# shao-lab/MotifScan

Hardware: AMD Instinct MI355X
Metric: scanned bp*motifs per second (region_bp x n_motifs), both strands, p=1e-4 cutoffs (higher is better)
Workload: dtype f64 (every hit decision and score, as in the reference) behind an fp6 x fp4 one-hot matrix-core pre-filter (exact f32 accumulate)

## Files before the change

include/motifscan_amd.h:

```cpp
#ifndef MOTIFSCAN_AMD_H
#define MOTIFSCAN_AMD_H

#include <stdint.h>

#ifdef __cplusplus
extern "C" {
#endif

#define MS_OK            0
#define MS_ERR_INVALID   1
#define MS_ERR_NOMEM     2
#define MS_ERR_RUNTIME   3

#define MS_STRAND_FWD    1
#define MS_STRAND_REV    2
#define MS_STRAND_BOTH   3

#define MS_SCAN_DEFAULT      0u
#define MS_SCAN_EXACT_ONLY   1u
#define MS_SCAN_COUNTS_ONLY  2u

typedef struct ms_pwmset ms_pwmset;
typedef struct ms_seqset ms_seqset;
typedef struct ms_result ms_result;
// ... 9 lines not shown
    int32_t n_tiles;
    int32_t n_passes;
    double  ms_prefilter;
    double  ms_exact;
    double  ms_sort;
    double  ms_finalize;
    double  ms_total;
    int64_t lds_bytes_read;
    int64_t hbm_bytes_algorithmic;
    double  pf_clock_mhz;
    int64_t mfma_ops;
    int64_t mfma_ops_algorithmic;
    int32_t pf_engine;
    int32_t order_overflow_runs;
    int32_t order_bucketed;
    int32_t reserved0;
} ms_scan_stats;

const char *ms_last_error(void);
int ms_version(void);

int ms_device_count(int *count);
int ms_set_device(int device);
int ms_device_name(char *buf, int buflen);
int ms_numa_bind_thread(int force, int *node);
int ms_device_pool_stats(uint64_t out[6]);

int ms_pwmset_create(const double *values, const int32_t *widths, const double *cutoffs,
                     int32_t n_pwms, ms_pwmset **out);
int ms_pwmset_set_cutoffs(ms_pwmset *pwms, const double *cutoffs);
int ms_pwmset_size(const ms_pwmset *pwms, int32_t *n_pwms);
// ... 161 lines not shown
```

include/motifscan_amd_debug.h:

```cpp
#ifndef MOTIFSCAN_AMD_DEBUG_H
#define MOTIFSCAN_AMD_DEBUG_H

#include "motifscan_amd.h"

#ifdef __cplusplus
extern "C" {
#endif

int ms_debug_plan_dims(const ms_pwmset *pwms, int strand_mask, int64_t lds_budget, int32_t *n_fast,
                       int32_t *n_exact, int32_t *n_groups, int32_t *n_tiles);

int ms_debug_plan_rows(const ms_pwmset *pwms, int32_t *group_fields, int16_t *rows, int32_t *bias, int32_t *group_kb,
                       int32_t *exact_motifs, int32_t *tile_first_group);

int ms_debug_host_pack(const char *bases, const int64_t *offsets, int64_t n_seqs, uint32_t *codes, uint32_t *nmask, int32_t *blk2reg, int32_t *blkinfo);

int ms_debug_numa_probe(const char *root, const char *bdf, int32_t *node, int32_t *n_cpus, int32_t *n_nodes);

int ms_debug_bucket_plan(const int64_t *offsets, int64_t n_seqs, const int32_t *widths, int32_t n_pwms, int32_t gbits, int32_t pbits, int32_t end_bit,
                         int32_t low_bits, int64_t n_regions, uint64_t *weights, double mu, uint64_t n_pred, uint64_t cap_max, uint32_t form, int32_t force,
                         uint64_t *need, int32_t *gate, uint64_t *base, uint64_t *cap);

int ms_debug_key_layout(int64_t n_bases, int64_t n_seqs, int64_t max_len, int32_t n_pwms, int32_t coord_global, int32_t *gbits, int32_t *pbits);

int ms_debug_release_scratch(void);

int ms_debug_varscan_chunk(int64_t n_variants, int64_t *previous);

int ms_debug_best_segment_windows(void);

int ms_debug_pair_lds_bins(void);
int ms_debug_cooc_chunk_regions(void);
int ms_debug_pair_lds_pair_limit(int64_t limit, int64_t *previous);

int ms_debug_plot_dims(int32_t out[6]);

// ... 11 lines not shown
```

motifscan_amd/_lib.py:

```python
import ctypes
import importlib.util
import os
import subprocess

import numpy as np

_HERE = os.path.dirname(os.path.abspath(__file__))
LIB_PATH = os.path.join(_HERE, "libmotifscan_amd.so")

MS_OK, MS_ERR_INVALID, MS_ERR_NOMEM, MS_ERR_RUNTIME = 0, 1, 2, 3
MS_SCAN_DEFAULT, MS_SCAN_EXACT_ONLY, MS_SCAN_COUNTS_ONLY = 0, 1, 2
MS_STREAM_DEDUP, MS_STREAM_NO_HITS, MS_STREAM_EXACT_ONLY, MS_STREAM_PACKED, MS_STREAM_HOST_PACK, MS_STREAM_PACKED12 = 1, 2, 4, 8, 16, 32
MS_PROFILE_UNSMOOTHED = 1
MS_REPLAY_DONE, MS_REPLAY_WORDS, MS_REPLAY_ATTEMPTS, MS_REPLAY_NO_SIZE, MS_REPLAY_EMPTY_RANGE, MS_REPLAY_WIDE = 0, 1, 2, 3, 4, 5
MS_REPLAY_SIZE_MISSING = -(1 << 63)


class ScanStats(ctypes.Structure):
    _fields_ = [("n_bases", ctypes.c_int64), ("n_windows", ctypes.c_int64), ("n_candidates", ctypes.c_int64),
                ("n_hits", ctypes.c_int64), ("n_pwms", ctypes.c_int32), ("n_pwms_exact", ctypes.c_int32),
                ("n_tiles", ctypes.c_int32), ("n_passes", ctypes.c_int32), ("ms_prefilter", ctypes.c_double),
                ("ms_exact", ctypes.c_double), ("ms_sort", ctypes.c_double), ("ms_finalize", ctypes.c_double),
                ("ms_total", ctypes.c_double), ("lds_bytes_read", ctypes.c_int64),
                ("hbm_bytes_algorithmic", ctypes.c_int64), ("pf_clock_mhz", ctypes.c_double),
                ("mfma_ops", ctypes.c_int64), ("mfma_ops_algorithmic", ctypes.c_int64), ("pf_engine", ctypes.c_int32),
                ("order_overflow_runs", ctypes.c_int32), ("order_bucketed", ctypes.c_int32), ("reserved0", ctypes.c_int32)]

    def as_dict(self):
        return {k: getattr(self, k) for k, _ in self._fields_}


class Span(ctypes.Structure):
    _fields_ = [("chrom", ctypes.c_int32), ("reserved", ctypes.c_int32), ("begin", ctypes.c_int64), ("end", ctypes.c_int64),
                ("first_window", ctypes.c_int64), ("n_windows", ctypes.c_int64)]


_lib = None


def build(verbose=False):
    cmd = ["make", "-C", os.path.join(_HERE, "csrc"), "-j4"]
# ... 133 lines not shown
        "ms_allelescan_num_sites": (c_int, [vp, pi64]),
        "ms_allelescan_motif_offsets": (c_int, [vp, pi64]),
        "ms_allelescan_sites": (c_int, [vp, pi64, pu8, pi64, pi8, pd]),
        "ms_allelescan_motif_counts": (c_int, [vp, pi64, pi64]),
        "ms_allelescan_ref_mismatch": (c_int, [vp, pu8]),
        "ms_allelescan_device_ms": (c_int, [vp, pd]),
        "ms_allelescan_free": (None, [vp]),
        "ms_scan_best": (c_int, [vp, vp, c_int, c_u32, pvp]),
        "ms_best_shape": (c_int, [vp, pi32, pi64]),
        "ms_best_sites": (c_int, [vp, c_i32, c_i32, pd, pi32, pi8]),
        "ms_best_sites_device": (c_int, [vp, pvp, pvp, pvp]),
        "ms_best_device_ms": (c_int, [vp, pd]),
        "ms_best_free": (None, [vp]),
        "ms_debug_best_segment_windows": (c_int, []),
        "ms_debug_key_layout": (c_int, [c_i64, c_i64, c_i64, c_i32, c_i32, pi32, pi32]),
    }
    for name, (res, args) in sig.items():
        fn = getattr(L, name)
        fn.restype, fn.argtypes = res, args
    _lib = L
    return L


def check(rc):
    if rc == MS_OK:
        return
    msg = lib().ms_last_error().decode("utf-8", "replace")
    if rc == MS_ERR_INVALID:
        raise ValueError(msg)
    if rc == MS_ERR_NOMEM:
# ... 584 lines not shown
    base, cap = np.zeros(256, dtype=np.uint64), np.zeros(256, dtype=np.uint64)
    form = (1 if predicted else 0) | (2 if counts_only else 0) | (4 if carry_only else 0) | (8 if sticky_off else 0)
    check(lib().ms_debug_bucket_plan(po, n_seqs, pw, n_pwms, int(gbits), int(pbits), int(end_bit), int(low_bits), int(n_regions), ptr(w, ctypes.c_uint64), float(mu),
                                     int(n_pred), (1 << 64) - 1 if cap_max is None else int(cap_max), form, int(force), ctypes.byref(need),
                                     ctypes.byref(gate), ptr(base, ctypes.c_uint64), ptr(cap, ctypes.c_uint64)))
    return {"weights": w, "need": need.value, "gate": bool(gate.value), "base": base, "cap": cap}


def key_layout(n_bases, n_seqs, max_len, n_pwms, coord_global=False):
    gbits, pbits = ctypes.c_int32(), ctypes.c_int32()
    check(lib().ms_debug_key_layout(int(n_bases), int(n_seqs), int(max_len), int(n_pwms), 1 if coord_global else 0, ctypes.byref(gbits),
                                    ctypes.byref(pbits)))
    return gbits.value, pbits.value


def host_pack(bases, offsets):
    bases = np.ascontiguousarray(bases, dtype=np.uint8)
    offsets = np.ascontiguousarray(offsets, dtype=np.int64)
    n = int(offsets[-1])
    units, blocks = (n + 31) // 32, (n + 63) // 64 + 1
    codes, nmask = np.zeros(2 * units, dtype=np.uint32), np.zeros(units, dtype=np.uint32)
    blk, info = np.zeros(blocks, dtype=np.int32), np.zeros((blocks, 4), dtype=np.int32)
    check(lib().ms_debug_host_pack(bases.ctypes.data_as(ctypes.c_char_p), ptr(offsets, ctypes.c_int64), offsets.size - 1,
                                   ptr(codes, ctypes.c_uint32), ptr(nmask, ctypes.c_uint32), ptr(blk, ctypes.c_int32), ptr(info, ctypes.c_int32)))
    return codes, nmask, blk, info


def host_pool_stats():
    out = (ctypes.c_uint64 * 4)()
    check(lib().ms_host_pool_stats(out))
# ... 518 lines not shown
```

motifscan_amd/csrc/ms_fp64.hip:

```cpp
#include "ms_device.h"

namespace ms {

__device__ __forceinline__ int64_t hit_coord(const HitOut &H, const DevSeq &S, int64_t r, int64_t g) {
    return H.pbits ? (int64_t) (((uint64_t) r << H.pbits) | (uint64_t) (g - S.offsets[r])) : g;
}

__device__ __forceinline__ void emit_hit(const HitOut &H, uint32_t motif, int64_t g, uint32_t sbit, double score) {
    const unsigned long long i = atomicAdd(H.n_hits, 1ULL);
    if (i < H.cap) {
        H.keys[i] = ((uint64_t) motif << (H.gbits + 1)) | ((uint64_t) g << 1) | sbit;
        H.vals[i] = score;
    }
}

__device__ __forceinline__ void test_and_emit(const HitOut &H, const DevPwm &Pw, uint32_t motif, int64_t g,
                                              double fwd, double rev, int strand_mask) {
    const double floor_ = Pw.raw_floor[motif];
    const bool try_f = (strand_mask & 1) && !(fwd < floor_);
    const bool try_r = (strand_mask & 2) && !(rev < floor_);
    if (!try_f && !try_r) return;
    const double max_raw = Pw.max_raw[motif];
    const double cutoff = Pw.cutoff[motif];
    const double s_f = try_f ? fwd / max_raw : 0.0, s_r = try_r ? rev / max_raw : 0.0;
// ... 35 lines not shown

template <class ST>
__device__ __forceinline__ void stage_flush(ST &st, const HitOut &H) {
    __syncthreads();
    const unsigned int n = st.n < (unsigned int) ST::kCap ? st.n : (unsigned int) ST::kCap;
    if (threadIdx.x == 0 && n > 0) st.base = atomicAdd(H.n_hits, (unsigned long long) n);
    __syncthreads();
    const unsigned long long base = st.base;
    for (unsigned int i = threadIdx.x; i < n; i += blockDim.x)
        if (base + i < H.cap) { H.keys[base + i] = st.keys[i]; H.vals[base + i] = st.vals[i]; }
    __syncthreads();
    if (threadIdx.x == 0) st.n = 0;
    __syncthreads();
}

template <class ST, class HO>
__device__ __forceinline__ void test_and_stage(ST &st, const HO &H, const DevPwm &Pw, uint32_t motif, int64_t g,
                                               double fwd, double rev, int strand_mask, float floor32) {
    const double floor_ = (double) floor32;
    const bool try_f = (strand_mask & 1) && !(fwd < floor_);
    const bool try_r = (strand_mask & 2) && !(rev < floor_);
    if (!try_f && !try_r) return;
    const double2 mc = *reinterpret_cast<const double2 *>(Pw.thresh + 4 * (size_t) motif);
    const double max_raw = mc.x, cutoff = mc.y;
    if (try_f) {
        const double s = fwd / max_raw;
        if (s - cutoff >= -1e-10) stage_hit(st, H, motif, g, 0u, s);
    }
    if (try_r) {
        const double s = rev / max_raw;
        if (s - cutoff >= -1e-10) stage_hit(st, H, motif, g, 1u, s);
    }
}

__global__ void __launch_bounds__(256) exact_all_kernel(const DevSeq S, const DevPwm Pw, const int32_t *__restrict__ motifs,
                                                        int strand_mask, const HitOut H) {
    const int64_t g = (int64_t) blockIdx.x * blockDim.x + threadIdx.x;
    if (g >= S.n_bases) return;
// ... 160 lines not shown
                       field_meta, strand_mask, H);
    MS_HIP(hipGetLastError());
    return MS_OK;
}

constexpr int kRwThreads = 1024;
constexpr int kRwPerThread = 4;
constexpr int kRwChunk = kRwThreads * kRwPerThread;
constexpr int kRwBins = 4096;
typedef HitStageN<2048> RwStage;
struct RwStageBk : RwStage {
    unsigned int cnt[kOrderBuckets], room[kOrderBuckets];
    unsigned long long lo[kOrderBuckets];
};

__device__ __forceinline__ void stage_flush(RwStageBk &st, const BucketHitOut &H) {
    constexpr int kPer = RwStageBk::kCap / kRwThreads;
    static_assert(kPer * kRwThreads == RwStageBk::kCap && kOrderBuckets <= kRwThreads, "stage_flush: one pass of the block over the stage");
    __syncthreads();
    const unsigned int n = st.n < (unsigned int) RwStageBk::kCap ? st.n : (unsigned int) RwStageBk::kCap;
    if (threadIdx.x < (unsigned int) kOrderBuckets) st.cnt[threadIdx.x] = 0;
    __syncthreads();
    uint32_t bk[kPer], rank[kPer];
#pragma unroll
    for (int k = 0; k < kPer; k++) {
        const unsigned int i = threadIdx.x + (unsigned int) (k * kRwThreads);
        bk[k] = i < n ? (uint32_t) (st.keys[i] >> H.B.shift) & 255u : 0u;
        rank[k] = i < n ? atomicAdd(&st.cnt[bk[k]], 1u) : 0u;
    }
    __syncthreads();
// ... 7 lines not shown
    }
    __syncthreads();
#pragma unroll
    for (int k = 0; k < kPer; k++) {
        const unsigned int i = threadIdx.x + (unsigned int) (k * kRwThreads);
        if (i < n && rank[k] < st.room[bk[k]]) {
            const unsigned long long at = st.lo[bk[k]] + rank[k];
            if (at < H.cap) { H.keys[at] = st.keys[i]; H.vals[at] = st.vals[i]; }
        }
    }
    __syncthreads();
    if (threadIdx.x == 0) st.n = 0;
    __syncthreads();
}

template <class HO, class ST>
__global__ void __launch_bounds__(kRwThreads) rescore_carry_kernel(const DevSeq S, const DevPwm Pw, const uint64_t *__restrict__ cand,
                                                                   const unsigned long long *__restrict__ n_cand, uint64_t n_static, uint64_t cand_cap,
                                                                   const FieldMeta *__restrict__ field_meta, int strand_mask, const HO H) {
    extern __shared__ uint4 rw_lds4[];
    uint64_t *s_cw = reinterpret_cast<uint64_t *>(rw_lds4);
    uint64_t *s_gk = s_cw + kRwChunk;
    uint32_t *s_nw = reinterpret_cast<uint32_t *>(s_gk + kRwChunk);
    uint32_t *s_gf = s_nw + kRwChunk;
    uint32_t *bins = s_gf + kRwChunk;
    uint32_t *wave_tot = bins + kRwBins;
    ST &st = *reinterpret_cast<ST *>(wave_tot + 32);
    if (threadIdx.x == 0) st.n = 0;
    unsigned long long n = n_static + *n_cand;
    if (n > cand_cap) n = cand_cap;
    const bool both = strand_mask == 3;
    const int4 *__restrict__ meta4 = reinterpret_cast<const int4 *>(field_meta);
    const uint32_t lane = threadIdx.x & 63u, wave = threadIdx.x >> 6;
    const uint64_t pmask = H.pbits ? ((1ULL << H.pbits) - 1ULL) : 0ULL;
    const unsigned long long n_chunks = (n + kRwChunk - 1) / kRwChunk;
    for (unsigned long long ch = blockIdx.x; ch < n_chunks; ch += gridDim.x) {
        for (uint32_t i = threadIdx.x; i < (uint32_t) kRwBins; i += kRwThreads) bins[i] = 0;
        __syncthreads();
        {
            uint64_t cw[kRwPerThread], gk[kRwPerThread];
            uint32_t nw[kRwPerThread], gf[kRwPerThread], key[kRwPerThread], rank[kRwPerThread];
            int64_t g[kRwPerThread];
            int4 bi[kRwPerThread];
#pragma unroll
            for (int k = 0; k < kRwPerThread; k++) {
                const unsigned long long i = ch * kRwChunk + (unsigned long long) k * kRwThreads + threadIdx.x;
                const uint64_t rec = i < n ? cand[i] : 0ULL;
                g[k] = (int64_t) (rec >> 30);
                gf[k] = (uint32_t) rec & 0x3FFFFFFFu;
                if (!(gf[k] & 0xFFFFu)) { gf[k] = 0; g[k] = 0; }
                bi[k] = S.blkinfo[g[k] >> 6];
                cw[k] = code_window(S.codes, g[k]);
                nw[k] = n_window(S.nmask, g[k]);
            }
#pragma unroll
            for (int k = 0; k < kRwPerThread; k++) {
                const int64_t base = g[k] & ~(int64_t) 63;
                int64_t lo = bi[k].x, o0 = base + bi[k].y, o1 = base + bi[k].z, o2 = base + bi[k].w, r, beg, end;
                if (bi[k].x < 0) {
                    lo = S.blk2reg[g[k] >> 6];
                    o0 = S.offsets[lo]; o1 = S.offsets[lo + 1];
                    o2 = lo + 2 <= S.R ? S.offsets[lo + 2] : o1;
                }
                if (g[k] < o1) { r = lo; beg = o0; end = o1; }
                else if (g[k] < o2) { r = lo + 1; beg = o1; end = o2; }
                else { r = find_region(S, g[k]); beg = S.offsets[r]; end = S.offsets[r + 1]; }
                const uint64_t coord = H.pbits ? (((uint64_t) r << H.pbits) | (uint64_t) (g[k] - beg)) : (uint64_t) g[k];
                const int64_t room = end - g[k];
                gk[k] = (coord << 8) | (uint64_t) (room > 255 ? 255 : (room < 0 ? 0 : room));
                const uint32_t f = gf[k] & 0xFFFFu;
                const uint32_t fl = both ? (f | (f >> 1)) & 0x5555u : f;
                key[k] = fl ? (((gf[k] >> 16) << 4) | (uint32_t) (__ffs((int) fl) - 1)) & (uint32_t) (kRwBins - 1) : (uint32_t) (kRwBins - 1);
            }
#pragma unroll
            for (int k = 0; k < kRwPerThread; k++) rank[k] = atomicAdd(&bins[key[k]], 1u);
            __syncthreads();
            {
                const uint32_t b0 = bins[4 * threadIdx.x], b1 = bins[4 * threadIdx.x + 1], b2 = bins[4 * threadIdx.x + 2], b3 = bins[4 * threadIdx.x + 3];
                const uint32_t tot = b0 + b1 + b2 + b3;
                uint32_t v = tot;
#pragma unroll
                for (int d = 1; d < 64; d <<= 1) {
                    const uint32_t o = __shfl_up(v, d);
                    if ((int) lane >= d) v += o;
                }
                if (lane == 63u) wave_tot[wave] = v;
                __syncthreads();
                uint32_t base = 0;
                for (uint32_t w = 0; w < wave; w++) base += wave_tot[w];
                const uint32_t excl = base + v - tot;
                bins[4 * threadIdx.x] = excl;
                bins[4 * threadIdx.x + 1] = excl + b0;
                bins[4 * threadIdx.x + 2] = excl + b0 + b1;
                bins[4 * threadIdx.x + 3] = excl + b0 + b1 + b2;
            }
            __syncthreads();
#pragma unroll
            for (int k = 0; k < kRwPerThread; k++) {
                const uint32_t at = bins[key[k]] + rank[k];
                s_cw[at] = cw[k]; s_gk[at] = gk[k]; s_nw[at] = nw[k]; s_gf[at] = gf[k];
            }
        }
        __syncthreads();
        for (int round = 0; round < 2; round++) {
#pragma unroll
            for (int u = 0; u < 2; u++) {
                const uint32_t at = (uint32_t) (round * 2 + u) * kRwThreads + threadIdx.x;
                const uint32_t gfu = s_gf[at];
                const uint32_t f = gfu & 0xFFFFu;
                uint32_t flags = both ? (f | (f >> 1)) & 0x5555u : f;
                if (!flags) continue;
                const uint64_t cwu = s_cw[at], gku = s_gk[at];
                const uint32_t nwu = s_nw[at];
                const int32_t group = (int32_t) (gfu >> 16);
                const int room = (int) (gku & 0xFFu);
                const int64_t coord = (int64_t) (gku >> 8);
                while (flags) {
                    const int field = __ffs((int) flags) - 1;
                    flags &= flags - 1u;
                    const int4 f4 = meta4[group * kGroupFields + field];
                    const int32_t m = f4.x;
                    const int w = f4.y;
                    if (m < 0) continue;
                    if (w > room) continue;
                    double fwd, rev;
                    if (w <= 32 && Pw.tab32) score_window32(Pw.tab2, (uint32_t) f4.z, Pw.zero_bytes, w, cwu, nwu, fwd, rev);
                    else {
                        const int64_t gpos = H.pbits ? S.offsets[coord >> H.pbits] + (int64_t) ((uint64_t) coord & pmask) : coord;
                        score_window(S, Pw.tab2 + Pw.tab_off[m], w, gpos, fwd, rev);
                    }
                    test_and_stage(st, H, Pw, (uint32_t) m, coord, fwd, rev, strand_mask, __int_as_float(f4.w));
                }
            }
            stage_flush(st, H);
        }
    }
}

template <class ST>
static size_t rescore_carry_lds_bytes() { return (size_t) kRwChunk * 24 + (size_t) kRwBins * 4 + 32 * 4 + sizeof(ST) + 64; }
int rescore_carry_set_lds() {
    MS_HIP(hipFuncSetAttribute(reinterpret_cast<const void *>(rescore_carry_kernel<HitOut, RwStage>), hipFuncAttributeMaxDynamicSharedMemorySize,
                               (int) rescore_carry_lds_bytes<RwStage>()));
    MS_HIP(hipFuncSetAttribute(reinterpret_cast<const void *>(rescore_carry_kernel<BucketHitOut, RwStageBk>), hipFuncAttributeMaxDynamicSharedMemorySize,
                               (int) rescore_carry_lds_bytes<RwStageBk>()));
    return MS_OK;
}
int launch_rescore_carry(const DevSeq &S, const DevPwm &Pw, const uint64_t *cand, const unsigned long long *n_cand, uint64_t n_static,
                         uint64_t cand_cap, const FieldMeta *field_meta, int strand_mask, const HitOut &H, int n_blocks, hipStream_t st) {
    hipLaunchKernelGGL((rescore_carry_kernel<HitOut, RwStage>), dim3((unsigned) n_blocks), dim3(kRwThreads), rescore_carry_lds_bytes<RwStage>(), st, S, Pw,
                       cand, n_cand, n_static, cand_cap, field_meta, strand_mask, H);
    MS_HIP(hipGetLastError());
    return MS_OK;
}
int launch_rescore_carry_bucketed(const DevSeq &S, const DevPwm &Pw, const uint64_t *cand, const unsigned long long *n_cand, uint64_t n_static,
                                  uint64_t cand_cap, const FieldMeta *field_meta, int strand_mask, const HitOut &H, const BucketOut &B, int n_blocks,
                                  hipStream_t st) {
    BucketHitOut HB;
    static_cast<HitOut &>(HB) = H;
    HB.B = B;
    hipLaunchKernelGGL((rescore_carry_kernel<BucketHitOut, RwStageBk>), dim3((unsigned) n_blocks), dim3(kRwThreads), rescore_carry_lds_bytes<RwStageBk>(), st,
                       S, Pw, cand, n_cand, n_static, cand_cap, field_meta, strand_mask, HB);
    MS_HIP(hipGetLastError());
    return MS_OK;
}

}
```

motifscan_amd/csrc/ms_kernels.h:

```cpp
#pragma once
#include "ms_internal.h"

namespace ms {

constexpr int kPfThreads = 1024;
constexpr int kPfBlocksPerCu = 1;
constexpr int kPfCounters = 8;
constexpr size_t kPfClsBytes = (size_t) kMaxClasses * 32;
constexpr size_t kF6LutBytes = 256 * 8 + kPfClsBytes;
constexpr int kPfStageWords = 24;
constexpr size_t kPfStageBytes = (size_t) (kPfThreads / 64) * kPfStageWords * sizeof(uint32_t);
constexpr int kRareCapMin = 16;
constexpr int kRareCapMax = 64;
constexpr int kRareEntryWords = 12;
constexpr size_t kPfRareBytesMin = (size_t) (kPfThreads / 64) * kRareCapMin * kRareEntryWords * sizeof(uint32_t);
constexpr size_t kPfOnehotBytes = (size_t) (kPfThreads / 64) * 160 * 16;
constexpr double kDenseHitsPerHalfTile = 12.0;
constexpr int kPfEmitWords = 16;
constexpr size_t kPfEmitBytes = (size_t) (kPfThreads / 64) * kPfEmitWords * sizeof(uint32_t);

struct DevSeq {
    const uint32_t *codes;
    const uint32_t *nmask;
    const int64_t *offsets;
// ... 68 lines not shown
    uint64_t cand_static;
    int skip_alln;
    unsigned int *chunk_counter;
    int use_counters;
    int wave_passes;
};

int prefilter_set_lds(bool wide, bool dense, size_t bytes);
int launch_prefilter(const PfArgs &A, bool wide, bool dense, int blocks_per_tile, int n_tiles, size_t lds_bytes, hipStream_t st);
int launch_exact_all(const DevSeq &S, const DevPwm &Pw, const int32_t *motifs, int32_t n_motifs, int strand_mask,
                     const HitOut &H, hipStream_t st, int max_width);
int launch_rescore(const DevSeq &S, const DevPwm &Pw, const uint64_t *cand, const unsigned long long *n_cand, uint64_t n_static,
                   uint64_t cand_cap, const FieldMeta *field_meta, int strand_mask, const HitOut &H, int n_blocks, hipStream_t st);
int rescore_carry_set_lds();
int launch_rescore_carry(const DevSeq &S, const DevPwm &Pw, const uint64_t *cand, const unsigned long long *n_cand, uint64_t n_static,
                         uint64_t cand_cap, const FieldMeta *field_meta, int strand_mask, const HitOut &H, int n_blocks, hipStream_t st);
int launch_rescore_carry_bucketed(const DevSeq &S, const DevPwm &Pw, const uint64_t *cand, const unsigned long long *n_cand, uint64_t n_static,
                                  uint64_t cand_cap, const FieldMeta *field_meta, int strand_mask, const HitOut &H, const BucketOut &B, int n_blocks,
                                  hipStream_t st);
int launch_fill_tail(uint64_t *keys, const unsigned long long *n_dev, uint64_t cap, hipStream_t st);
int launch_bucket_plan(const BucketWeights &bw, double mu, unsigned long long n_pred, unsigned long long need, unsigned long long cap_max,
                       unsigned long long *tab, hipStream_t st);
int launch_fill_tail_buckets(uint64_t *keys, const unsigned long long *tab, uint64_t n_pred, unsigned long long *n_hits, unsigned long long *overflow,
                             hipStream_t st);
int launch_sort_fixup(uint64_t *keys, double *vals, int64_t n, const unsigned long long *n_dev, hipStream_t st);
int launch_finalize(const uint64_t *keys, int64_t n, const unsigned long long *n_dev, int gbits, int rbits, int pbits, int32_t P, const DevSeq &S,
                    int64_t *seq_idx, int64_t *pos, int8_t *strand, int64_t *motif_first, unsigned long long *region_counts,
                    hipStream_t st);
size_t order_overflow_bytes(size_t n, int run_cap);
int launch_order_finalize(uint64_t *keys, double *score, int64_t n, const unsigned long long *n_dev, int L, int rbits, int pbits, int32_t P,
                          int64_t *seq_idx, int64_t *pos, int8_t *strand, int64_t *motif_first, unsigned long long *region_counts,
                          uint64_t *tmp_keys, double *tmp_vals, void *ovf_buf, size_t ovf_bytes, unsigned long long *ovf_n, int run_cap,
                          hipStream_t st);
bool count_only_supported(int32_t P, int64_t R, int pbits);
// ... 8 lines not shown
```

motifscan_amd/csrc/ms_scan.hip:

```cpp
#include <algorithm>
#include <cmath>
#include <climits>
#include <cstring>
#include <memory>
#include <mutex>

#include "ms_handles.h"
#include "ms_scan_geom.h"

namespace ms {

static int scratch_reserve(Scratch &sc, size_t cand_cap, size_t hit_cap) {
    int rc;
    if (cand_cap > sc.cand_cap) {
        dev_free(sc.cand);
        sc.cand_cap = 0;
        if ((rc = dev_alloc(&sc.cand, cand_cap))) return rc;
        sc.cand_cap = cand_cap;
    }
    if (hit_cap > sc.hit_cap) {
        dev_free(sc.keys); dev_free(sc.vals); dev_free(sc.keys_sorted);
        sc.hit_cap = 0;
        if ((rc = dev_alloc(&sc.keys, hit_cap))) return rc;
        if ((rc = dev_alloc(&sc.vals, hit_cap))) return rc;
// ... 99 lines not shown


struct ScanCtx {
    DeviceCtx *c = nullptr;
    ms_pwmset *pwms = nullptr;
    const ms_seqset *seqs = nullptr;
    ms_result *raw = nullptr;
    int strand_mask = 3;
    uint32_t flags = 0;
    ScanKey key;
    ScanGeom g;
    hipEvent_t *ev = nullptr;
    DevSeq S;
    DevPwm Pw;
    bool counts_ok = false;
    bool bucketed = false;
    int bk_L = 0;
    double bk_mu = 0.0;
    unsigned long long bk_need = 0, bk_cap_max = ~0ULL;
    BucketWeights bk_w;
};

static int scan_plan(DeviceCtx *c, ms_pwmset *pwms, const ScanKey &key, const ScanOverrides &ov) {
    int rc;
    bool may_be_wide = false, wide = false;
    for (int32_t w : pwms->widths) may_be_wide = may_be_wide || (w >= 2 * kF6Cols && w <= kMaxFastWidth);
    if (may_be_wide && !key.exact_only && !(pwms->narrow_key == key)) {
        if ((rc = pwmset_plan(pwms, key.strand, scan_lds_budget(c->lds_max, true, ov), key.exact_only, false, c->device))) return rc;
        wide = pwms->plan.wide;
        if (!wide) pwms->narrow_key = key;
// ... 95 lines not shown
}

static int scan_front(ScanCtx &x, const HitOut &H, const BucketOut *B = nullptr) {
    DeviceCtx *c = x.c;
    Scratch &sc = c->sc;
    const PrefilterPlan &plan = x.pwms->plan;
    int rc;
    hipError_t he = hipMemsetAsync(sc.counters, 0, 8 * sizeof(unsigned long long), c->stream);
    if (he != hipSuccess) { set_error("memset failed: %s", hipGetErrorString(he)); return MS_ERR_RUNTIME; }
    (void) hipEventRecord(x.ev[0], c->stream);
    if (x.g.n_tiles > 0 && (rc = scan_prefilter(x))) return rc;
    (void) hipEventRecord(x.ev[1], c->stream);
    if (!plan.fast_motifs.empty()) {
        if (x.g.rescore_carry) {
            if (!c->rc_lds_set) { if ((rc = rescore_carry_set_lds())) return rc; c->rc_lds_set = true; }
            if (B) rc = launch_rescore_carry_bucketed(x.S, x.Pw, sc.cand, sc.counters, x.g.cand_static, sc.cand_cap, x.pwms->d_field_meta, x.strand_mask, H, *B, c->n_cu, c->stream);
            else rc = launch_rescore_carry(x.S, x.Pw, sc.cand, sc.counters, x.g.cand_static, sc.cand_cap, x.pwms->d_field_meta, x.strand_mask, H, c->n_cu, c->stream);
            if (rc) return rc;
        } else if ((rc = launch_rescore(x.S, x.Pw, sc.cand, sc.counters, x.g.cand_static, sc.cand_cap, x.pwms->d_field_meta, x.strand_mask, H, c->n_cu * 8, c->stream))) return rc;
    }
    if (!plan.exact_motifs.empty()) {
        int max_w = 0;
        for (int32_t m : plan.exact_motifs) max_w = std::max(max_w, (int) x.pwms->widths[m]);
        if ((rc = launch_exact_all(x.S, x.Pw, x.pwms->d_exact_motifs, (int32_t) plan.exact_motifs.size(), x.strand_mask, H, c->stream, max_w))) return rc;
    }
    (void) hipEventRecord(x.ev[2], c->stream);
    return MS_OK;
}

static bool scan_counts_fast(const ScanCtx &x, size_t n_expected) {
    return x.counts_ok && (double) x.pwms->P * (double) x.seqs->R <= 50.0 * (double) std::max<size_t>(n_expected, 1);
}
// ... 216 lines not shown
    std::unique_ptr<ms_result, void (*)(ms_result *)> res(scan_result_new(c, pwms, seqs, strand_mask, &sh.fast_windows), ms_result_free);
    if (!res) return MS_ERR_NOMEM;
    x.raw = res.get();
    if (pwms->P == 0 || seqs->n_bases == 0) {
        if ((rc = scan_empty(x))) return rc;
        *out = res.release();
        return MS_OK;
    }

    const bool density_known = pwms->pred_density >= 0 && pwms->pred_key == x.key;
    sh.plan = &pwms->plan; sh.P = pwms->P;
    sh.n_bases = seqs->n_bases; sh.R = seqs->R; sh.max_len = seqs->len_sorted.empty() ? 0 : seqs->len_sorted.back();
    sh.n_cu = c->n_cu; sh.lds_max = c->lds_max; sh.cu_reserved = c->n_streams.load() > 0 ? c->n_cu_copy : 0;
    sh.density_known = density_known; sh.pred_density = pwms->pred_density;
    x.g = scan_geometry(sh, ov);
    x.S = dev_seq(seqs);
    x.Pw = dev_pwm(pwms);
    x.counts_ok = (flags & MS_SCAN_COUNTS_ONLY_INTERNAL) && !(flags & MS_SCAN_RAW_INTERNAL) && count_only_supported(pwms->P, seqs->R, x.g.pbits);
    ms_scan_stats &stt = x.raw->stats;
    if (x.g.n_tiles > 0 && x.g.dense) stt.pf_engine = 4;

    Scratch &sc = c->sc;
    size_t want_cand = x.g.want_cand, want_hits = x.g.want_hits;
    if (density_known && !(flags & (MS_SCAN_RAW_INTERNAL | MS_SCAN_NO_PREDICT_INTERNAL)) && !ov.no_predict) {
        if (pend) x.ev = pend->ev;
        const double mu = pwms->pred_density * (double) stt.n_windows;
        size_t n_pred = (size_t) std::min<double>(mu * (1.0 + pwms->pred_margin) + 6.0 * std::sqrt(mu + 1.0) + 256.0, 3.0e9);
        scan_bucket_decide(x, ov, mu, &n_pred);
        if ((rc = scan_queue_predicted(x, n_pred, pend != nullptr))) return rc;
        if (pend) {
// ... 59 lines not shown
        for (int b = 0; b < kOrderBuckets; b++) { bw.w[b] = weights[b]; bw.total += weights[b]; }
    }
    BucketShape bs;
    bs.predicted = (form & 1u) != 0; bs.counts_only = (form & 2u) != 0; bs.carry_only = (form & 4u) != 0; bs.sticky_off = (form & 8u) != 0;
    bs.pbits = pbits; bs.gbits = gbits; bs.end_bit = end_bit; bs.L = low_bits; bs.P = n_pwms; bs.R = offsets ? n_seqs : n_regions;
    ScanOverrides ov;
    ov.order_buckets = force < 0 ? -1 : (force ? 1 : 0);
    *need = bucket_need(bw, mu);
    *gate = bw.total > 0 && bucket_gate(bs, ov, *need, n_pred) ? 1 : 0;
    unsigned long long b64[kOrderBuckets], c64[kOrderBuckets];
    bucket_caps(bw, mu, n_pred, cap_max, b64, c64);
    for (int b = 0; b < kOrderBuckets; b++) { base[b] = b64[b]; cap[b] = c64[b]; }
    return MS_OK;
}

int ms_debug_key_layout(int64_t n_bases, int64_t n_seqs, int64_t max_len, int32_t n_pwms, int32_t coord_global, int32_t *gbits, int32_t *pbits) {
    if (!gbits || !pbits) { set_error("NULL argument"); return MS_ERR_INVALID; }
    if (n_bases < 0 || n_seqs < 0 || max_len < 0 || max_len > n_bases || n_pwms < 0) { set_error("invalid sizes"); return MS_ERR_INVALID; }
    const ScanGeom g = scan_key_layout(n_bases, n_seqs, max_len, n_pwms, coord_global != 0);
    *gbits = g.gbits;
    *pbits = g.pbits;
    return MS_OK;
}

}
```

motifscan_amd/csrc/ms_scan_geom.cpp:

```cpp
#include <algorithm>
#include <cmath>
#include <vector>

#include "ms_scan_geom.h"

namespace ms {

ScanOverrides read_scan_overrides() {
    ScanOverrides o;
    if (const char *e = measure_env("MS_PF_LDS_BUDGET")) o.lds_budget = (size_t) std::max(1, atoi(e));
    if (const char *e = measure_env("MS_PF_DENSE")) o.pf_dense = atoi(e) != 0 ? 1 : 0;
    if (const char *e = measure_env("MS_PF_RARE_CAP")) o.rare_cap_max = std::max(kRareCapMin, atoi(e));
    if (const char *e = measure_env("MS_PF_MAX_BLOCKS")) o.max_blocks = std::max(1, atoi(e));
    if (const char *e = measure_env("MS_HIT_COORD")) o.coord_global = e[0] == 'g';
    if (const char *e = measure_env("MS_RESCORE_SORTED_MIN")) o.rescore_sorted_min = atof(e);
    o.sort_full = measure_env("MS_SORT_FULL") != nullptr;
    if (const char *e = measure_env("MS_SORT_LOW_BITS")) o.sort_low_bits = std::max(0, atoi(e));
    if (const char *e = measure_env("MS_ORDER_RUN_CAP")) o.order_run_cap = std::max(1, atoi(e));
    if (const char *e = measure_env("MS_SORT_FIXUP_MIN")) o.fixup_min = (size_t) std::max(0, atoi(e));
    o.no_predict = measure_env("MS_NO_PREDICT") != nullptr;
    if (const char *e = measure_env("MS_ORDER_BUCKETS")) o.order_buckets = atoi(e) != 0 ? 1 : 0;
    if (const char *e = measure_env("MS_ORDER_BUCKET_CAP")) o.bucket_cap_max = (uint64_t) std::max(0LL, atoll(e));
    return o;
}

size_t scan_lds_budget(size_t lds_max, bool wide, const ScanOverrides &ov) {
    return std::min(lds_max / (size_t) kPfBlocksPerCu - (wide ? kPfLdsFixedWide : kPfLdsFixedNarrow), ov.lds_budget);
}

static int bits_for(int64_t n) {
// ... 182 lines not shown
```

motifscan_amd/csrc/ms_scan_geom.h:

```cpp
#pragma once
#include <climits>
#include <cmath>

#include "ms_kernels.h"

namespace ms {

struct ScanOverrides {
    size_t lds_budget = (size_t) -1;
    int pf_dense = -1;
    int rare_cap_max = kRareCapMax;
    int max_blocks = INT_MAX;
    bool coord_global = false;
    double rescore_sorted_min = 2.0e6;
    bool sort_full = false;
    int sort_low_bits = -1;
    int order_run_cap = 1 << 30;
    size_t fixup_min = (size_t) 1 << 20;
    bool no_predict = false;
    int order_buckets = -1;
    uint64_t bucket_cap_max = ~0ULL;
};
MS_HIDDEN ScanOverrides read_scan_overrides();

constexpr size_t kPfLdsFixedWide = kF6LutBytes + kPfStageBytes + kPfEmitBytes + kPfRareBytesMin;
constexpr size_t kPfLdsFixedNarrow = kPfLdsFixedWide + kPfOnehotBytes;
MS_HIDDEN size_t scan_lds_budget(size_t lds_max, bool wide, const ScanOverrides &ov);

struct ScanShape {
// ... 51 lines not shown
```

Before: 14810 billion.

## Cache field metadata and motif thresholds in LDS for rescore carry kernel

The rescore-carry kernel now stages per-group field metadata and per-motif max/cutoff pairs into LDS when they fit within a 160 KiB budget, instead of reading them from global memory for every candidate. Bins now alias the stage keys to free LDS space. The kernel also adds a batched fixed-width column scoring path that issues all table loads before accumulating, and swaps the scan's shfl_up for ds_bpermute. The trade-off is a larger dynamic LDS allocation, which may lower occupancy, plus extra template instantiations and an early exit for blocks with no chunks.

```diff
diff --git a/include/motifscan_amd.h b/include/motifscan_amd.h
--- a/include/motifscan_amd.h
+++ b/include/motifscan_amd.h
@@ -47,7 +47,7 @@
     int32_t pf_engine;
     int32_t order_overflow_runs;
     int32_t order_bucketed;
-    int32_t reserved0;
+    int32_t rescore_lds_meta;
 } ms_scan_stats;
 
 const char *ms_last_error(void);
diff --git a/include/motifscan_amd_debug.h b/include/motifscan_amd_debug.h
--- a/include/motifscan_amd_debug.h
+++ b/include/motifscan_amd_debug.h
@@ -20,6 +20,8 @@
 int ms_debug_bucket_plan(const int64_t *offsets, int64_t n_seqs, const int32_t *widths, int32_t n_pwms, int32_t gbits, int32_t pbits, int32_t end_bit,
                          int32_t low_bits, int64_t n_regions, uint64_t *weights, double mu, uint64_t n_pred, uint64_t cap_max, uint32_t form, int32_t force,
                          uint64_t *need, int32_t *gate, uint64_t *base, uint64_t *cap);
+
+int ms_debug_rescore_lds_fit(int32_t n_groups, int32_t n_pwms, int32_t strand_mask, int32_t bucketed, int64_t *need, int64_t *free_bytes, int32_t *fits);
 
 int ms_debug_key_layout(int64_t n_bases, int64_t n_seqs, int64_t max_len, int32_t n_pwms, int32_t coord_global, int32_t *gbits, int32_t *pbits);
 
diff --git a/motifscan_amd/_lib.py b/motifscan_amd/_lib.py
--- a/motifscan_amd/_lib.py
+++ b/motifscan_amd/_lib.py
@@ -24,7 +24,7 @@
                 ("ms_total", ctypes.c_double), ("lds_bytes_read", ctypes.c_int64),
                 ("hbm_bytes_algorithmic", ctypes.c_int64), ("pf_clock_mhz", ctypes.c_double),
                 ("mfma_ops", ctypes.c_int64), ("mfma_ops_algorithmic", ctypes.c_int64), ("pf_engine", ctypes.c_int32),
-                ("order_overflow_runs", ctypes.c_int32), ("order_bucketed", ctypes.c_int32), ("reserved0", ctypes.c_int32)]
+                ("order_overflow_runs", ctypes.c_int32), ("order_bucketed", ctypes.c_int32), ("rescore_lds_meta", ctypes.c_int32)]
 
     def as_dict(self):
         return {k: getattr(self, k) for k, _ in self._fields_}
@@ -188,6 +188,7 @@
         "ms_best_free": (None, [vp]),
         "ms_debug_best_segment_windows": (c_int, []),
         "ms_debug_key_layout": (c_int, [c_i64, c_i64, c_i64, c_i32, c_i32, pi32, pi32]),
+        "ms_debug_rescore_lds_fit": (c_int, [c_i32, c_i32, c_i32, c_i32, pi64, pi64, pi32]),
     }
     for name, (res, args) in sig.items():
         fn = getattr(L, name)
@@ -802,6 +803,13 @@
     return gbits.value, pbits.value
 
 
+def rescore_lds_fit(n_groups, n_pwms, strand_mask=3, bucketed=False):
+    need, free, fits = ctypes.c_int64(), ctypes.c_int64(), ctypes.c_int32()
+    check(lib().ms_debug_rescore_lds_fit(int(n_groups), int(n_pwms), int(strand_mask), 1 if bucketed else 0, ctypes.byref(need),
+                                         ctypes.byref(free), ctypes.byref(fits)))
+    return {"need": need.value, "free": free.value, "fits": bool(fits.value)}
+
+
 def host_pack(bases, offsets):
     bases = np.ascontiguousarray(bases, dtype=np.uint8)
     offsets = np.ascontiguousarray(offsets, dtype=np.int64)
diff --git a/motifscan_amd/csrc/ms_fp64.hip b/motifscan_amd/csrc/ms_fp64.hip
--- a/motifscan_amd/csrc/ms_fp64.hip
+++ b/motifscan_amd/csrc/ms_fp64.hip
@@ -1,4 +1,13 @@
+#include <algorithm>
+
 #include "ms_device.h"
+
+#ifndef MS_RW_BATCH
+#define MS_RW_BATCH 12
+#endif
+#ifndef MS_RW_PREFETCH
+#define MS_RW_PREFETCH 0
+#endif
 
 namespace ms {
 
@@ -73,14 +82,14 @@
     __syncthreads();
 }
 
-template <class ST, class HO>
+template <bool LM = false, class ST, class HO>
 __device__ __forceinline__ void test_and_stage(ST &st, const HO &H, const DevPwm &Pw, uint32_t motif, int64_t g,
-                                               double fwd, double rev, int strand_mask, float floor32) {
+                                               double fwd, double rev, int strand_mask, float floor32, const double2 *mc_lds = nullptr) {
     const double floor_ = (double) floor32;
     const bool try_f = (strand_mask & 1) && !(fwd < floor_);
     const bool try_r = (strand_mask & 2) && !(rev < floor_);
     if (!try_f && !try_r) return;
-    const double2 mc = *reinterpret_cast<const double2 *>(Pw.thresh + 4 * (size_t) motif);
+    const double2 mc = LM ? mc_lds[motif] : *reinterpret_cast<const double2 *>(Pw.thresh + 4 * (size_t) motif);
     const double max_raw = mc.x, cutoff = mc.y;
     if (try_f) {
         const double s = fwd / max_raw;
@@ -271,6 +280,10 @@
     unsigned long long lo[kOrderBuckets];
 };
 
+constexpr size_t kRwLdsMax = 160 * 1024;
+template <class ST>
+constexpr size_t kRwMetaOff = ((size_t) kRwChunk * 24 + 32 * 4 + sizeof(ST) + 64 + 15) & ~(size_t) 15;
+
 __device__ __forceinline__ void stage_flush(RwStageBk &st, const BucketHitOut &H) {
     constexpr int kPer = RwStageBk::kCap / kRwThreads;
     static_assert(kPer * kRwThreads == RwStageBk::kCap && kOrderBuckets <= kRwThreads, "stage_flush: one pass of the block over the stage");
@@ -308,26 +321,73 @@
     __syncthreads();
 }
 
-template <class HO, class ST>
+constexpr int kRwBatchW = MS_RW_BATCH ? MS_RW_BATCH : 12;
+template <int N>
+__device__ __forceinline__ void score_columns_batch(const char *__restrict__ base, uint32_t t0, uint32_t zero_bytes, uint32_t bits, uint32_t sk, double &fwd, double &rev) {
+    double2 t[N];
+#pragma unroll
+    for (int k = 0; k < N; k++) {
+        const uint32_t off = t0 + (uint32_t) k * 64u + ((bits >> (2 * k)) & 3u) * 16u;
+        const uint32_t sel = (uint32_t) -(int32_t) ((sk >> k) & 1u);
+        t[k] = *reinterpret_cast<const double2 *>(base + ((off & ~sel) | (zero_bytes & sel)));
+    }
+    asm volatile("" ::: "memory");
+    __builtin_amdgcn_sched_barrier(0);
+#pragma unroll
+    for (int k = 0; k < N; k++) {
+        fwd += t[k].x;
+        rev += t[k].y;
+    }
+}
+__device__ __forceinline__ void score_window_batch(const double2 *__restrict__ tab2, uint32_t tab_bytes, uint32_t zero_bytes, int W, uint64_t cw, uint32_t nw,
+                                                   double &fwd, double &rev) {
+    fwd = 0.0;
+    rev = 0.0;
+    const uint32_t skip = nw | ~low_mask(W);
+    const char *__restrict__ base = reinterpret_cast<const char *>(tab2);
+    const uint32_t bits = (uint32_t) cw;
+    if (W <= 4) score_columns_batch<4>(base, tab_bytes, zero_bytes, bits, skip, fwd, rev);
+    else if (W <= 8) score_columns_batch<8>(base, tab_bytes, zero_bytes, bits, skip, fwd, rev);
+    else if (W <= 12 || kRwBatchW < 16) score_columns_batch<12>(base, tab_bytes, zero_bytes, bits, skip, fwd, rev);
+    else score_columns_batch<16>(base, tab_bytes, zero_bytes, bits, skip, fwd, rev);
+}
+
+template <class HO, class ST, bool LM>
 __global__ void __launch_bounds__(kRwThreads) rescore_carry_kernel(const DevSeq S, const DevPwm Pw, const uint64_t *__restrict__ cand,
                                                                    const unsigned long long *__restrict__ n_cand, uint64_t n_static, uint64_t cand_cap,
-                                                                   const FieldMeta *__restrict__ field_meta, int strand_mask, const HO H) {
+                                                                   const FieldMeta *__restrict__ field_meta, int n_groups, int strand_mask, const HO H) {
     extern __shared__ uint4 rw_lds4[];
     uint64_t *s_cw = reinterpret_cast<uint64_t *>(rw_lds4);
     uint64_t *s_gk = s_cw + kRwChunk;
     uint32_t *s_nw = reinterpret_cast<uint32_t *>(s_gk + kRwChunk);
     uint32_t *s_gf = s_nw + kRwChunk;
-    uint32_t *bins = s_gf + kRwChunk;
-    uint32_t *wave_tot = bins + kRwBins;
+    uint32_t *wave_tot = s_gf + kRwChunk;
     ST &st = *reinterpret_cast<ST *>(wave_tot + 32);
-    if (threadIdx.x == 0) st.n = 0;
+    static_assert(sizeof(st.keys) >= sizeof(uint32_t) * kRwBins, "the bins alias the stage's keys");
+    uint32_t *bins = reinterpret_cast<uint32_t *>(st.keys);
+    int4 *s_meta = reinterpret_cast<int4 *>(reinterpret_cast<char *>(rw_lds4) + kRwMetaOff<ST>);
     unsigned long long n = n_static + *n_cand;
     if (n > cand_cap) n = cand_cap;
     const bool both = strand_mask == 3;
     const int4 *__restrict__ meta4 = reinterpret_cast<const int4 *>(field_meta);
-    const uint32_t lane = threadIdx.x & 63u, wave = threadIdx.x >> 6;
+    const uint32_t n_meta = (uint32_t) n_groups * (both ? (uint32_t) kGroupFields / 2u : (uint32_t) kGroupFields);
+    double2 *s_mc = reinterpret_cast<double2 *>(s_meta + n_meta);
     const uint64_t pmask = H.pbits ? ((1ULL << H.pbits) - 1ULL) : 0ULL;
     const unsigned long long n_chunks = (n + kRwChunk - 1) / kRwChunk;
+    if (blockIdx.x >= n_chunks) return;
+    if (threadIdx.x == 0) st.n = 0;
+    if (LM) {
+        for (uint32_t i = threadIdx.x; i < n_meta; i += kRwThreads) s_meta[i] = meta4[both ? (i >> 3) * (uint32_t) kGroupFields + (i & 7u) * 2u : i];
+        for (uint32_t i = threadIdx.x; i < (uint32_t) Pw.P; i += kRwThreads) s_mc[i] = *reinterpret_cast<const double2 *>(Pw.thresh + 4 * (size_t) i);
+    }
+#if MS_RW_PREFETCH
+    uint64_t rec[kRwPerThread];
+#pragma unroll
+    for (int k = 0; k < kRwPerThread; k++) {
+        const unsigned long long i = (unsigned long long) blockIdx.x * kRwChunk + (unsigned long long) k * kRwThreads + threadIdx.x;
+        rec[k] = i < n ? cand[i] : 0ULL;
+    }
+#endif
     for (unsigned long long ch = blockIdx.x; ch < n_chunks; ch += gridDim.x) {
         for (uint32_t i = threadIdx.x; i < (uint32_t) kRwBins; i += kRwThreads) bins[i] = 0;
         __syncthreads();
@@ -338,15 +398,26 @@
             int4 bi[kRwPerThread];
 #pragma unroll
             for (int k = 0; k < kRwPerThread; k++) {
+#if MS_RW_PREFETCH
+                const uint64_t r_ = rec[k];
+#else
                 const unsigned long long i = ch * kRwChunk + (unsigned long long) k * kRwThreads + threadIdx.x;
-                const uint64_t rec = i < n ? cand[i] : 0ULL;
-                g[k] = (int64_t) (rec >> 30);
-                gf[k] = (uint32_t) rec & 0x3FFFFFFFu;
+                const uint64_t r_ = i < n ? cand[i] : 0ULL;
+#endif
+                g[k] = (int64_t) (r_ >> 30);
+                gf[k] = (uint32_t) r_ & 0x3FFFFFFFu;
                 if (!(gf[k] & 0xFFFFu)) { gf[k] = 0; g[k] = 0; }
                 bi[k] = S.blkinfo[g[k] >> 6];
                 cw[k] = code_window(S.codes, g[k]);
                 nw[k] = n_window(S.nmask, g[k]);
             }
+#if MS_RW_PREFETCH
+#pragma unroll
+            for (int k = 0; k < kRwPerThread; k++) {
+                const unsigned long long i = (ch + gridDim.x) * kRwChunk + (unsigned long long) k * kRwThreads + threadIdx.x;
+                rec[k] = i < n ? cand[i] : 0ULL;
+            }
+#endif
 #pragma unroll
             for (int k = 0; k < kRwPerThread; k++) {
                 const int64_t base = g[k] & ~(int64_t) 63;
@@ -370,23 +441,26 @@
             for (int k = 0; k < kRwPerThread; k++) rank[k] = atomicAdd(&bins[key[k]], 1u);
             __syncthreads();
             {
-                const uint32_t b0 = bins[4 * threadIdx.x], b1 = bins[4 * threadIdx.x + 1], b2 = bins[4 * threadIdx.x + 2], b3 = bins[4 * threadIdx.x + 3];
+                uint32_t tid = threadIdx.x;
+                asm volatile("" : "+v"(tid));
+                const uint32_t ln = tid & 63u, wv = tid >> 6;
+                const uint32_t b0 = bins[4 * tid], b1 = bins[4 * tid + 1], b2 = bins[4 * tid + 2], b3 = bins[4 * tid + 3];
                 const uint32_t tot = b0 + b1 + b2 + b3;
                 uint32_t v = tot;
 #pragma unroll
                 for (int d = 1; d < 64; d <<= 1) {
-                    const uint32_t o = __shfl_up(v, d);
-                    if ((int) lane >= d) v += o;
+                    const uint32_t o = (uint32_t) __builtin_amdgcn_ds_bpermute((int) ((ln - (uint32_t) d) << 2), (int) v);
+                    if ((int) ln >= d) v += o;
                 }
-                if (lane == 63u) wave_tot[wave] = v;
+                if (ln == 63u) wave_tot[wv] = v;
                 __syncthreads();
                 uint32_t base = 0;
-                for (uint32_t w = 0; w < wave; w++) base += wave_tot[w];
+                for (uint32_t w = 0; w < wv; w++) base += wave_tot[w];
                 const uint32_t excl = base + v - tot;
-                bins[4 * threadIdx.x] = excl;
-                bins[4 * threadIdx.x + 1] = excl + b0;
-                bins[4 * threadIdx.x + 2] = excl + b0 + b1;
-                bins[4 * threadIdx.x + 3] = excl + b0 + b1 + b2;
+                bins[4 * tid] = excl;
+                bins[4 * tid + 1] = excl + b0;
+                bins[4 * tid + 2] = excl + b0 + b1;
+                bins[4 * tid + 3] = excl + b0 + b1 + b2;
             }
             __syncthreads();
 #pragma unroll
@@ -412,18 +486,23 @@
                 while (flags) {
                     const int field = __ffs((int) flags) - 1;
                     flags &= flags - 1u;
-                    const int4 f4 = meta4[group * kGroupFields + field];
+                    const int4 f4 = LM ? s_meta[both ? group * (kGroupFields / 2) + (field >> 1) : group * kGroupFields + field]
+                                       : meta4[group * kGroupFields + field];
                     const int32_t m = f4.x;
                     const int w = f4.y;
                     if (m < 0) continue;
                     if (w > room) continue;
                     double fwd, rev;
+#if MS_RW_BATCH
+                    if (w <= kRwBatchW && Pw.tab32) score_window_batch(Pw.tab2, (uint32_t) f4.z, Pw.zero_bytes, w, cwu, nwu, fwd, rev);
+                    else
+#endif
                     if (w <= 32 && Pw.tab32) score_window32(Pw.tab2, (uint32_t) f4.z, Pw.zero_bytes, w, cwu, nwu, fwd, rev);
                     else {
                         const int64_t gpos = H.pbits ? S.offsets[coord >> H.pbits] + (int64_t) ((uint64_t) coord & pmask) : coord;
                         score_window(S, Pw.tab2 + Pw.tab_off[m], w, gpos, fwd, rev);
                     }
-                    test_and_stage(st, H, Pw, (uint32_t) m, coord, fwd, rev, strand_mask, __int_as_float(f4.w));
+                    test_and_stage<LM>(st, H, Pw, (uint32_t) m, coord, fwd, rev, strand_mask, __int_as_float(f4.w), s_mc);
                 }
             }
             stage_flush(st, H);
@@ -431,32 +510,56 @@
     }
 }
 
+RescoreLdsFit rescore_lds_fit(int64_t n_groups, int64_t P, int strand_mask, bool bucketed) {
+    RescoreLdsFit f;
+    const int64_t fields = strand_mask == 3 ? kGroupFields / 2 : kGroupFields;
+    f.need = std::max<int64_t>(n_groups, 0) * fields * (int64_t) sizeof(FieldMeta) + std::max<int64_t>(P, 0) * (int64_t) sizeof(double2);
+    f.free = (int64_t) kRwLdsMax - (int64_t) (bucketed ? kRwMetaOff<RwStageBk> : kRwMetaOff<RwStage>);
+    f.fits = f.need <= f.free;
+    return f;
+}
+
 template <class ST>
-static size_t rescore_carry_lds_bytes() { return (size_t) kRwChunk * 24 + (size_t) kRwBins * 4 + 32 * 4 + sizeof(ST) + 64; }
+static size_t rescore_carry_lds_bytes(const RescoreLdsFit &f) { return kRwMetaOff<ST> + (f.fits ? (size_t) f.need : 0); }
+template <class HO, class ST, bool LM>
+static int rescore_carry_raise_lds() {
+    MS_HIP(hipFuncSetAttribute(reinterpret_cast<const void *>(rescore_carry_kernel<HO, ST, LM>), hipFuncAttributeMaxDynamicSharedMemorySize, (int) kRwLdsMax));
+    return MS_OK;
+}
 int rescore_carry_set_lds() {
-    MS_HIP(hipFuncSetAttribute(reinterpret_cast<const void *>(rescore_carry_kernel<HitOut, RwStage>), hipFuncAttributeMaxDynamicSharedMemorySize,
-                               (int) rescore_carry_lds_bytes<RwStage>()));
-    MS_HIP(hipFuncSetAttribute(reinterpret_cast<const void *>(rescore_carry_kernel<BucketHitOut, RwStageBk>), hipFuncAttributeMaxDynamicSharedMemorySize,
-                               (int) rescore_carry_lds_bytes<RwStageBk>()));
+    int rc;
+    if ((rc = rescore_carry_raise_lds<HitOut, RwStage, false>()) || (rc = rescore_carry_raise_lds<HitOut, RwStage, true>())) return rc;
+    if ((rc = rescore_carry_raise_lds<BucketHitOut, RwStageBk, false>()) || (rc = rescore_carry_raise_lds<BucketHitOut, RwStageBk, true>())) return rc;
     return MS_OK;
 }
-int launch_rescore_carry(const DevSeq &S, const DevPwm &Pw, const uint64_t *cand, const unsigned long long *n_cand, uint64_t n_static,
-                         uint64_t cand_cap, const FieldMeta *field_meta, int strand_mask, const HitOut &H, int n_blocks, hipStream_t st) {
-    hipLaunchKernelGGL((rescore_carry_kernel<HitOut, RwStage>), dim3((unsigned) n_blocks), dim3(kRwThreads), rescore_carry_lds_bytes<RwStage>(), st, S, Pw,
-                       cand, n_cand, n_static, cand_cap, field_meta, strand_mask, H);
+template <class HO, class ST>
+static int launch_carry(const DevSeq &S, const DevPwm &Pw, const uint64_t *cand, const unsigned long long *n_cand, uint64_t n_static, uint64_t cand_cap,
+                        const FieldMeta *field_meta, int n_groups, int strand_mask, const HO &H, bool bucketed, int n_blocks, hipStream_t st, bool *lds_meta) {
+    RescoreLdsFit f = rescore_lds_fit(n_groups, Pw.P, strand_mask, bucketed);
+    f.fits = f.fits && *lds_meta;
+    *lds_meta = f.fits;
+    const size_t lds = rescore_carry_lds_bytes<ST>(f);
+    if (f.fits)
+        hipLaunchKernelGGL((rescore_carry_kernel<HO, ST, true>), dim3((unsigned) n_blocks), dim3(kRwThreads), lds, st, S, Pw, cand, n_cand, n_static, cand_cap,
+                           field_meta, n_groups, strand_mask, H);
+    else
+        hipLaunchKernelGGL((rescore_carry_kernel<HO, ST, false>), dim3((unsigned) n_blocks), dim3(kRwThreads), lds, st, S, Pw, cand, n_cand, n_static, cand_cap,
+                           field_meta, n_groups, strand_mask, H);
     MS_HIP(hipGetLastError());
     return MS_OK;
 }
+int launch_rescore_carry(const DevSeq &S, const DevPwm &Pw, const uint64_t *cand, const unsigned long long *n_cand, uint64_t n_static,
+                         uint64_t cand_cap, const FieldMeta *field_meta, int n_groups, int strand_mask, const HitOut &H, int n_blocks, hipStream_t st,
+                         bool *lds_meta) {
+    return launch_carry<HitOut, RwStage>(S, Pw, cand, n_cand, n_static, cand_cap, field_meta, n_groups, strand_mask, H, false, n_blocks, st, lds_meta);
+}
 int launch_rescore_carry_bucketed(const DevSeq &S, const DevPwm &Pw, const uint64_t *cand, const unsigned long long *n_cand, uint64_t n_static,
-                                  uint64_t cand_cap, const FieldMeta *field_meta, int strand_mask, const HitOut &H, const BucketOut &B, int n_blocks,
-                                  hipStream_t st) {
+                                  uint64_t cand_cap, const FieldMeta *field_meta, int n_groups, int strand_mask, const HitOut &H, const BucketOut &B,
+                                  int n_blocks, hipStream_t st, bool *lds_meta) {
     BucketHitOut HB;
     static_cast<HitOut &>(HB) = H;
     HB.B = B;
-    hipLaunchKernelGGL((rescore_carry_kernel<BucketHitOut, RwStageBk>), dim3((unsigned) n_blocks), dim3(kRwThreads), rescore_carry_lds_bytes<RwStageBk>(), st,
-                       S, Pw, cand, n_cand, n_static, cand_cap, field_meta, strand_mask, HB);
-    MS_HIP(hipGetLastError());
-    return MS_OK;
-}
-
-}
+    return launch_carry<BucketHitOut, RwStageBk>(S, Pw, cand, n_cand, n_static, cand_cap, field_meta, n_groups, strand_mask, HB, true, n_blocks, st, lds_meta);
+}
+
+}
diff --git a/motifscan_amd/csrc/ms_kernels.h b/motifscan_amd/csrc/ms_kernels.h
--- a/motifscan_amd/csrc/ms_kernels.h
+++ b/motifscan_amd/csrc/ms_kernels.h
@@ -106,10 +106,16 @@
                    uint64_t cand_cap, const FieldMeta *field_meta, int strand_mask, const HitOut &H, int n_blocks, hipStream_t st);
 int rescore_carry_set_lds();
 int launch_rescore_carry(const DevSeq &S, const DevPwm &Pw, const uint64_t *cand, const unsigned long long *n_cand, uint64_t n_static,
-                         uint64_t cand_cap, const FieldMeta *field_meta, int strand_mask, const HitOut &H, int n_blocks, hipStream_t st);
+                         uint64_t cand_cap, const FieldMeta *field_meta, int n_groups, int strand_mask, const HitOut &H, int n_blocks, hipStream_t st,
+                         bool *lds_meta);
 int launch_rescore_carry_bucketed(const DevSeq &S, const DevPwm &Pw, const uint64_t *cand, const unsigned long long *n_cand, uint64_t n_static,
-                                  uint64_t cand_cap, const FieldMeta *field_meta, int strand_mask, const HitOut &H, const BucketOut &B, int n_blocks,
-                                  hipStream_t st);
+                                  uint64_t cand_cap, const FieldMeta *field_meta, int n_groups, int strand_mask, const HitOut &H, const BucketOut &B,
+                                  int n_blocks, hipStream_t st, bool *lds_meta);
+struct RescoreLdsFit {
+    int64_t need = 0, free = 0;
+    bool fits = false;
+};
+RescoreLdsFit rescore_lds_fit(int64_t n_groups, int64_t P, int strand_mask, bool bucketed);
 int launch_fill_tail(uint64_t *keys, const unsigned long long *n_dev, uint64_t cap, hipStream_t st);
 int launch_bucket_plan(const BucketWeights &bw, double mu, unsigned long long n_pred, unsigned long long need, unsigned long long cap_max,
                        unsigned long long *tab, hipStream_t st);
diff --git a/motifscan_amd/csrc/ms_scan.hip b/motifscan_amd/csrc/ms_scan.hip
--- a/motifscan_amd/csrc/ms_scan.hip
+++ b/motifscan_amd/csrc/ms_scan.hip
@@ -137,6 +137,8 @@
     DevSeq S;
     DevPwm Pw;
     bool counts_ok = false;
+    int rescore_blocks = INT_MAX;
+    bool rescore_lds_meta = true;
     bool bucketed = false;
     int bk_L = 0;
     double bk_mu = 0.0;
@@ -262,8 +264,11 @@
     if (!plan.fast_motifs.empty()) {
         if (x.g.rescore_carry) {
             if (!c->rc_lds_set) { if ((rc = rescore_carry_set_lds())) return rc; c->rc_lds_set = true; }
-            if (B) rc = launch_rescore_carry_bucketed(x.S, x.Pw, sc.cand, sc.counters, x.g.cand_static, sc.cand_cap, x.pwms->d_field_meta, x.strand_mask, H, *B, c->n_cu, c->stream);
-            else rc = launch_rescore_carry(x.S, x.Pw, sc.cand, sc.counters, x.g.cand_static, sc.cand_cap, x.pwms->d_field_meta, x.strand_mask, H, c->n_cu, c->stream);
+            const int n_groups = (int) (plan.group_fields.size() / kGroupFields), n_blocks = std::max(1, std::min(c->n_cu, x.rescore_blocks));
+            bool lds_meta = x.rescore_lds_meta;
+            if (B) rc = launch_rescore_carry_bucketed(x.S, x.Pw, sc.cand, sc.counters, x.g.cand_static, sc.cand_cap, x.pwms->d_field_meta, n_groups, x.strand_mask, H, *B, n_blocks, c->stream, &lds_meta);
+            else rc = launch_rescore_carry(x.S, x.Pw, sc.cand, sc.counters, x.g.cand_static, sc.cand_cap, x.pwms->d_field_meta, n_groups, x.strand_mask, H, n_blocks, c->stream, &lds_meta);
+            x.raw->stats.rescore_lds_meta = lds_meta ? 1 : 0;
             if (rc) return rc;
         } else if ((rc = launch_rescore(x.S, x.Pw, sc.cand, sc.counters, x.g.cand_static, sc.cand_cap, x.pwms->d_field_meta, x.strand_mask, H, c->n_cu * 8, c->stream))) return rc;
     }
@@ -510,6 +515,8 @@
     sh.n_cu = c->n_cu; sh.lds_max = c->lds_max; sh.cu_reserved = c->n_streams.load() > 0 ? c->n_cu_copy : 0;
     sh.density_known = density_known; sh.pred_density = pwms->pred_density;
     x.g = scan_geometry(sh, ov);
+    x.rescore_blocks = ov.rescore_blocks;
+    x.rescore_lds_meta = ov.rescore_lds_meta;
     x.S = dev_seq(seqs);
     x.Pw = dev_pwm(pwms);
     x.counts_ok = (flags & MS_SCAN_COUNTS_ONLY_INTERNAL) && !(flags & MS_SCAN_RAW_INTERNAL) && count_only_supported(pwms->P, seqs->R, x.g.pbits);
@@ -599,6 +606,16 @@
     return MS_OK;
 }
 
+int ms_debug_rescore_lds_fit(int32_t n_groups, int32_t n_pwms, int32_t strand_mask, int32_t bucketed, int64_t *need, int64_t *free_bytes, int32_t *fits) {
+    if (!need || !free_bytes || !fits) { set_error("NULL argument"); return MS_ERR_INVALID; }
+    if (n_groups < 0 || n_pwms < 0 || strand_mask < 1 || strand_mask > 3) { set_error("invalid sizes"); return MS_ERR_INVALID; }
+    const RescoreLdsFit f = rescore_lds_fit(n_groups, n_pwms, strand_mask, bucketed != 0);
+    *need = f.need;
+    *free_bytes = f.free;
+    *fits = f.fits ? 1 : 0;
+    return MS_OK;
+}
+
 int ms_debug_key_layout(int64_t n_bases, int64_t n_seqs, int64_t max_len, int32_t n_pwms, int32_t coord_global, int32_t *gbits, int32_t *pbits) {
     if (!gbits || !pbits) { set_error("NULL argument"); return MS_ERR_INVALID; }
     if (n_bases < 0 || n_seqs < 0 || max_len < 0 || max_len > n_bases || n_pwms < 0) { set_error("invalid sizes"); return MS_ERR_INVALID; }
diff --git a/motifscan_amd/csrc/ms_scan_geom.cpp b/motifscan_amd/csrc/ms_scan_geom.cpp
--- a/motifscan_amd/csrc/ms_scan_geom.cpp
+++ b/motifscan_amd/csrc/ms_scan_geom.cpp
@@ -14,6 +14,8 @@
     if (const char *e = measure_env("MS_PF_MAX_BLOCKS")) o.max_blocks = std::max(1, atoi(e));
     if (const char *e = measure_env("MS_HIT_COORD")) o.coord_global = e[0] == 'g';
     if (const char *e = measure_env("MS_RESCORE_SORTED_MIN")) o.rescore_sorted_min = atof(e);
+    if (const char *e = measure_env("MS_RESCORE_LDS_META")) o.rescore_lds_meta = atoi(e) != 0;
+    if (const char *e = measure_env("MS_RESCORE_BLOCKS")) o.rescore_blocks = std::max(1, atoi(e));
     o.sort_full = measure_env("MS_SORT_FULL") != nullptr;
     if (const char *e = measure_env("MS_SORT_LOW_BITS")) o.sort_low_bits = std::max(0, atoi(e));
     if (const char *e = measure_env("MS_ORDER_RUN_CAP")) o.order_run_cap = std::max(1, atoi(e));
diff --git a/motifscan_amd/csrc/ms_scan_geom.h b/motifscan_amd/csrc/ms_scan_geom.h
--- a/motifscan_amd/csrc/ms_scan_geom.h
+++ b/motifscan_amd/csrc/ms_scan_geom.h
@@ -13,6 +13,8 @@
     int max_blocks = INT_MAX;
     bool coord_global = false;
     double rescore_sorted_min = 2.0e6;
+    bool rescore_lds_meta = true;
+    int rescore_blocks = INT_MAX;
     bool sort_full = false;
     int sort_low_bits = -1;
     int order_run_cap = 1 << 30;
```

Measured after the change: 14860 billion, median of 6. No clear change (+0.4%).
